# Edward-Sun/DIFUSCO

Hardware: AMD Instinct MI355X
Metric: denoising steps/sec (graphs x steps / s), TSP-1000 k-NN sparse categorical (higher is better)
Workload: dtype f32 (fp16x3 split MFMA, fp32 accumulate)

## Files before the change

difusco_amd/_lib.py:

```python
import ctypes
import os

from .build import LIB_PATH, PROF_LIB_PATH

FLAG_NO_L0_FOLD, FLAG_NO_TAIL_FOLD, FLAG_CHECK_FINITE = 1, 2, 4

ABI_VERSION = 13
TASK_TSP, TASK_MIS = 0, 1
CATEGORICAL, GAUSSIAN = 0, 1
RAND_NONE, RAND_INJECTED, RAND_PHILOX, RAND_PHILOX_INSTANCES = 0, 1, 2, 3
PREC_FP32, PREC_BF16X3, PREC_BF16X6, PREC_FP16X3, PREC_FP16X1 = 0, 1, 2, 3, 4
PRECISIONS = {"fp32": PREC_FP32, "bf16x3": PREC_BF16X3, "bf16x6": PREC_BF16X6, "fp16x3": PREC_FP16X3,
              "fp16x1": PREC_FP16X1}
FUSED_PRECISIONS = ("bf16x3", "fp16x3", "fp16x1")
GRAPH_PERM_IDENTITY, GRAPH_ORDER_IDENTITY, GRAPH_BAD_EDGE = 1, 2, 4
AGGREGATIONS = {"sum": 0, "mean": 1, "max": 2}

W_GLOBAL = ["node_embed.weight", "node_embed.bias", "edge_embed.weight", "edge_embed.bias",
            "time_embed.0.weight", "time_embed.0.bias", "time_embed.2.weight", "time_embed.2.bias",
            "out.0.weight", "out.0.bias", "out.2.weight", "out.2.bias",
            "@time_freqs", "@dimt_pos", "@dimt_scalar", "@planes:edge_embed.weight"]
W_LAYER = ["@node4.weight", "@node4.bias", "layers.{l}.C.weight", "layers.{l}.C.bias",
           "layers.{l}.norm_h.weight", "layers.{l}.norm_h.bias", "layers.{l}.norm_e.weight", "layers.{l}.norm_e.bias",
           "time_embed_layers.{l}.1.weight", "time_embed_layers.{l}.1.bias",
# ... 145 lines not shown
```

difusco_amd/csrc/api.hip:

```cpp
#include <hip/hip_runtime.h>

#include <cstdarg>
#include <cstdio>
#include <cstring>
#include <mutex>
#include <vector>

#include "../../include/difusco_hip.h"
#include "kernels.h"

namespace {

thread_local char g_err[512] = "";

int fail(int code, const char* fmt, ...) {
  va_list ap;
  va_start(ap, fmt);
  vsnprintf(g_err, sizeof(g_err), fmt, ap);
  va_end(ap);
  return code;
}

#define HIP_TRY(expr)                                                                         \
  do {                                                                                        \
// ... 195 lines not shown
  if (a->n_layers < 1) return fail(DIFUSCO_EINVAL, "n_layers must be >= 1");
  if (a->out_channels != 1 && a->out_channels != 2) return fail(DIFUSCO_EINVAL, "out_channels must be 1 or 2 (got %d)", a->out_channels);
  if (a->precision < DIFUSCO_PREC_FP32 || a->precision > DIFUSCO_PREC_FP16X1) return fail(DIFUSCO_EINVAL, "unknown precision %d", a->precision);
  return DIFUSCO_OK;
}

struct StepPlan {
  int H, L, C;
  int64_t N, E, out_rows, E_pad, n_tiles_pad;
  bool tsp, head_only;
  int nprec;
  bool f16;
  bool fused;
  int fused_variant;
  bool l0_fold, tail_fold, gn_fold, use_prep;
};

StepPlan make_plan(const difusco_step_args* a) {
  StepPlan p;
  p.H = a->hidden, p.L = a->n_layers, p.C = a->out_channels;
  p.N = a->n_nodes, p.E = a->n_edges;
  p.tsp = a->task == DIFUSCO_TASK_TSP;
  p.out_rows = p.tsp ? p.E : p.N;
  p.head_only = a->gn_phase == 2;
  p.nprec = a->precision == DIFUSCO_PREC_FP16X1 ? DIFUSCO_PREC_FP16X3 : a->precision;
  p.f16 = p.nprec == DIFUSCO_PREC_FP16X3;
  const int reg_gather = p.N >= (1 << 20) ? 1 : 0;
  const bool agg_max = a->aggregation == DIFUSCO_AGG_MAX;
  p.fused = p.H == 256 && !a->no_fusion && p.E > 0 && !(agg_max && reg_gather) &&
            (a->precision == DIFUSCO_PREC_BF16X3 || a->precision == DIFUSCO_PREC_FP16X3 ||
             a->precision == DIFUSCO_PREC_FP16X1);
  p.fused_variant = reg_gather | (agg_max ? 2 : 0);
  p.E_pad = (p.E + 255) / 256 * 256;
  p.n_tiles_pad = p.E_pad / 32;
#ifdef DIFUSCO_PROFILING
  const bool ablating = difusco::g_fused_ablate != 0;
#else
  const bool ablating = false;
#endif
  p.l0_fold = p.fused && (a->flags & DIFUSCO_FLAG_NO_L0_FOLD) == 0 && !ablating && (p.tsp ? a->xt_is_binary != 0 : true);
  p.tail_fold = p.fused && p.L >= 2 && (a->flags & DIFUSCO_FLAG_NO_TAIL_FOLD) == 0 && !ablating;
  p.gn_fold = p.tail_fold && p.tsp;
  p.use_prep = a->prepared != nullptr && p.fused && p.tsp && !ablating;
  return p;
}

hipError_t time_bias_rows(const Weights& w, int H, int L, const float* t_host, int n_t, float* out, hipStream_t st) {
  const int64_t* l0 = w.lo.off.data() + DIFUSCO_W_GLOBAL_COUNT;
  return difusco::launch_time_bias(t_host, n_t, H, L, w.g(DIFUSCO_W_TIME_FREQS), w.g(DIFUSCO_W_TIME0_W), w.g(DIFUSCO_W_TIME0_B),
                                   w.g(DIFUSCO_W_TIME2_W), w.g(DIFUSCO_W_TIME2_B), w.base + l0[0], w.lo.layer_stride,
                                   l0[DIFUSCO_WL_TIME_W] - l0[0], l0[DIFUSCO_WL_TIME_B] - l0[0], out, st);
}

int embed_tsp_nodes(const Weights& w, int H, int64_t N, const float* points, float* feat, float* h0, hipStream_t st, bool prof) {
  PROF_IF(prof, PROF_EMBED, launch_pos_embed(points, w.g(DIFUSCO_W_DIMT_POS), (int)N, H, feat, st))
  PROF_IF(prof, PROF_LINEAR_NODE, linear_rows(feat, w.g(DIFUSCO_W_NODE_EMBED_W), w.g(DIFUSCO_W_NODE_EMBED_B), nullptr, h0, N, H, H, H, st))
  return DIFUSCO_OK;
}

int node_rows(int precision, int H, int64_t N, const LayerW& lw, const float* h, float* hscale, bool scale_pass, bool fused_domain,
              float* dst, hipStream_t st, bool prof) {
  const int nprec = precision == DIFUSCO_PREC_FP16X1 ? DIFUSCO_PREC_FP16X3 : precision;
  const bool f16 = nprec == DIFUSCO_PREC_FP16X3;
  bool converted = false;
  if (precision != DIFUSCO_PREC_FP32 && H == 256) {
    const SplitPlanes np = split_planes(lw.node4_planes, 4 * H, H, f16);
    SplitScale sc;
    if (f16) {
      if (scale_pass) PROF_IF(prof, PROF_LINEAR_NODE, launch_row_pow2_scale(h, N, H, hscale, st))
      sc.row_scale = hscale;
      sc.w_inv = np.w_inv;
    }
    converted = fused_domain && (nprec == DIFUSCO_PREC_BF16X3 || nprec == DIFUSCO_PREC_FP16X3);
    if (converted) sc.w_inv = lw.node4_fused_s + (f16 ? 0 : 4 * H);
    PROF_IF(prof, PROF_LINEAR_NODE, linear_rows_split(h, np.planes, (long long)4 * H * H, nprec, converted ? lw.node4_fused_b : lw.node4_b,
                                                      nullptr, dst, N, H, 4 * H, 4 * H, st, 0, sc))
  } else {
    PROF_IF(prof, PROF_LINEAR_NODE, linear_rows(h, lw.node4_w, lw.node4_b, nullptr, dst, N, H, 4 * H, 4 * H, st))
  }
  if (fused_domain && !converted && H == 256) PROF_IF(prof, PROF_LINEAR_NODE, launch_fuse_node_tables(dst, lw.c_b, (int)N, dst, st))
  return DIFUSCO_OK;
}

hipError_t table_c_rows(int precision, int H, float* table, const LayerW& lw, float* scale2, hipStream_t st) {
  if (precision != DIFUSCO_PREC_FP16X1) return launch_two_rows_linear(H, table, lw.c_w, nullptr, table + 2 * H, st);
  hipError_t er = launch_row_pow2_scale(table, 2, H, scale2, st);
  if (er != hipSuccess) return er;
  const SplitPlanes cp = split_planes(lw.c_planes, H, H, true);
  SplitScale sc;
  sc.row_scale = scale2;
  sc.w_inv = cp.w_inv;
// ... 63 lines not shown
  }

  int embed_mis() const {
    PROF(PROF_EMBED, launch_scalar_embed(a->xt, nullptr, w.g(DIFUSCO_W_DIMT_SCALAR), p.N, H, ws.node4, st))
    PROF(PROF_LINEAR_NODE, linear_rows(ws.node4, w.g(DIFUSCO_W_NODE_EMBED_W), w.g(DIFUSCO_W_NODE_EMBED_B), nullptr, ws.h, p.N, H, H, H, st))
    if (p.l0_fold) {
      PROF(PROF_EMBED, zero_async(ws.table, sizeof(float) * 4 * H, st))
      PROF(PROF_EMBED, zero_pad_tail())
    } else if (p.E > 0) {
      PROF(PROF_EMBED, zero_async(ws.e, sizeof(float) * (p.fused ? p.E_pad : p.E) * H, st))
      if (p.fused && p.f16) PROF(PROF_EMBED, zero_async(ws.etmax, sizeof(float) * p.n_tiles_pad, st))
    }
    return DIFUSCO_OK;
  }

  int fused_layer(int l, const LayerW& lw, const float* node4, const float* h_in) const {
    const float* tb = tbias + (size_t)l * H;
    FusedLayerArgs fa;
    fa.e = ws.e, fa.node4 = node4, fa.row = a->row, fa.col = a->col, fa.n_edges = (int)p.E;
    fa.c_planes = split_planes(lw.c_planes, H, H, p.f16).planes;
    fa.o_planes = split_planes(lw.out_planes, H, H, p.f16).planes;
    fa.plane_stride = (long long)H * H;
    fa.b_c = lw.c_b, fa.g_e = lw.norm_e_w, fa.b_e = lw.norm_e_b, fa.tbias = tb;
    fa.g_o = lw.out_ln_w, fa.b_o = lw.out_ln_b, fa.b_out = lw.out_b;
    fa.time_on_edge = p.tsp ? 1 : 0;
    fa.part = ws.part, fa.direct = ws.direct, fa.scales = lw.fused_scales, fa.stream = st;
    FusedKind kind = FusedKind::Middle;
    if (l == 0 && p.l0_fold) {
      kind = FusedKind::FirstFromTable;
      fa.l0_table = table, fa.l0_x = p.tsp ? a->xt : nullptr, fa.l0_perm = p.tsp ? a->perm : nullptr;
      fa.etmax_out = ws.etmax;
    } else if (p.tail_fold && l == p.L - 1) {
      kind = p.tsp ? FusedKind::TailTsp : FusedKind::TailMis;
      fa.gn_tile = ws.gn_tile, fa.etmax_in = ws.etmax;
    } else {
      fa.etmax_in = fa.etmax_out = ws.etmax;
    }
    PROF(PROF_LINEAR_EDGE, launch_edge_layer_fused(a->precision, kind, p.fused_variant, fa))
    if (p.gn_fold && l == p.L - 1) return DIFUSCO_OK;
#ifdef DIFUSCO_PROFILING
    if (g_step_skip & 1) return DIFUSCO_OK;
#endif
    PROF(PROF_GATE, launch_node_finalize((int)p.N, (int)p.E, a->rowptr, node4, ws.part, ws.direct, ws.h, lw.norm_h_w, lw.norm_h_b, tb,
                                         p.tsp ? 1 : 0, p.f16 ? ws.hscale : nullptr, st, h_in, a->aggregation))
    return DIFUSCO_OK;
  }

  int unfused_layer(int l, const LayerW& lw) const {
    PROF(PROF_LINEAR_EDGE, edge_linear(a->precision, ws.e, lw.c_w, lw.c_planes, lw.c_b, nullptr, ws.tmp))
    PROF(PROF_GATE, launch_edge_gate_aggregate(H, (int)p.N, a->rowptr, a->col, ws.node4, ws.tmp, ws.h, lw.norm_h_w, lw.norm_h_b,
                                               lw.norm_e_w, lw.norm_e_b, lw.out_ln_w, lw.out_ln_b, tbias + (size_t)l * H,
                                               p.tsp ? 1 : 0, st, a->aggregation))
    PROF(PROF_LINEAR_EDGE, edge_linear(a->precision, ws.tmp, lw.out_w, lw.out_planes, lw.out_b, ws.e, ws.e))
    return DIFUSCO_OK;
  }

  int run_layers() const {
    for (int l = 0; l < p.L; ++l) {
      const LayerW lw = w.layer(l);
      const bool prep_l = p.use_prep && l == 0;
      bool node_linear = !prep_l;
#ifdef DIFUSCO_PROFILING
      if ((g_step_skip & 2) && l >= 2) node_linear = false;
#endif
      if (node_linear)
        STAGE(node_rows(a->precision, H, p.N, lw, ws.h, ws.hscale, !p.fused || l == 0, p.fused, ws.node4, st, true));
      STAGE(p.fused ? fused_layer(l, lw, prep_l ? prep.node4_0 : ws.node4, prep_l ? prep.h0 : nullptr) : unfused_layer(l, lw));
    }
    return DIFUSCO_OK;
  }

  int run_head(const uint64_t* offset_shift) const {
    RandInstances ri;
    if (a->rand_mode == DIFUSCO_RAND_PHILOX_INSTANCES) ri = RandInstances{a->n_instances, a->instance_rows, a->instance_seeds};
    const int* seg_ptr = a->n_segments > 1 ? a->seg_ptr : nullptr;
    const int nblk = gn_blocks_for(p.out_rows);
    if (p.fused && p.tsp) {
      PROF(PROF_HEAD, launch_head_tiled(p.C, ws.e, p.E, nblk < 8 ? 8 : nblk / 8 * 8, ws.partial, ws.stats, w.g(DIFUSCO_W_OUT_GN_W),
                                        w.g(DIFUSCO_W_OUT_GN_B), w.g(DIFUSCO_W_OUT_CONV_W), w.g(DIFUSCO_W_OUT_CONV_B), a->perm, a->xt,
                                        a->post, a->rand_mode, a->rand, a->seed, a->offset, a->xt_out, a->pred_out, a->prob_out, st,
                                        p.gn_fold ? ws.gn_tile : nullptr, a->gn_phase, a->gn_sums, seg_ptr, a->n_segments, ri,
                                        offset_shift))
      return DIFUSCO_OK;
    }
    PROF(PROF_HEAD, launch_head(H, p.C, p.tsp ? ws.e : ws.h, seg_ptr, a->n_segments, p.out_rows, nblk, ws.partial, ws.stats,
                                w.g(DIFUSCO_W_OUT_GN_W), w.g(DIFUSCO_W_OUT_GN_B), w.g(DIFUSCO_W_OUT_CONV_W), w.g(DIFUSCO_W_OUT_CONV_B),
                                p.tsp ? a->perm : nullptr, a->xt, a->post, a->rand_mode, a->rand, a->seed, a->offset, a->xt_out,
                                a->pred_out, a->prob_out, st, a->gn_phase, a->gn_sums, ri, offset_shift))
    return DIFUSCO_OK;
  }

  int check_finite() const {
    if ((a->flags & DIFUSCO_FLAG_CHECK_FINITE) == 0 || a->gn_phase == 1) return DIFUSCO_OK;
    unsigned* cnt = reinterpret_cast<unsigned*>(ws.partial);
    HIP_TRY(hipMemsetAsync(cnt, 0, sizeof(unsigned), st));
    HIP_TRY(launch_count_nonfinite(a->xt_out, p.out_rows, cnt, st));
    HIP_TRY(launch_count_nonfinite(ws.stats, (long long)a->n_segments * 64, cnt, st));
// ... 382 lines not shown
```

difusco_amd/csrc/graph_kernels.hip:

```cpp
#include "common.h"
#include "kernels.h"

namespace difusco {

template <int VEC>
struct Vec {
  float v[VEC];
};

template <int VEC>
__device__ __forceinline__ Vec<VEC> ldv(const float* p) {
  Vec<VEC> r;
  if constexpr (VEC == 4) {
    const v4f t = *reinterpret_cast<const v4f*>(p);
    r.v[0] = t[0]; r.v[1] = t[1]; r.v[2] = t[2]; r.v[3] = t[3];
  } else if constexpr (VEC == 2) {
    typedef float v2f __attribute__((ext_vector_type(2)));
    const v2f t = *reinterpret_cast<const v2f*>(p);
    r.v[0] = t[0]; r.v[1] = t[1];
  } else {
    r.v[0] = *p;
  }
  return r;
}
// ... 212 lines not shown
  }
  s += __shfl_xor(s, 1, 64);
  q += __shfl_xor(q, 1, 64);
  if ((lane & 1) == 0) {
    red[wave][lane >> 1][0] = s;
    red[wave][lane >> 1][1] = q;
  }
  __syncthreads();
  if (threadIdx.x < 64) {
    const int g = threadIdx.x >> 1, w = threadIdx.x & 1;
    const double t = red[0][g][w] + red[1][g][w] + red[2][g][w] + red[3][g][w];
    partial[((long long)seg * gridDim.x + blockIdx.x) * 64 + g * 2 + w] = t;
  }
}

__global__ __launch_bounds__(1024) void gn_finalize_kernel(const double* __restrict__ partial, const int* __restrict__ seg_ptr,
                                                          long long total_rows, int nblk, int ch_per_group,
                                                          int group_stride_blocks, float* __restrict__ stats,
                                                          double* __restrict__ sums_out) {
  __shared__ double red[16][64];
  const int seg = blockIdx.x;
  const int c = threadIdx.x >> 6, gw = threadIdx.x & 63, g = gw >> 1, nch = blockDim.x >> 6;
  double acc = 0.0;
  if (group_stride_blocks == 1) {
    for (int b = c; b < nblk; b += nch) acc += partial[((long long)seg * nblk + b) * 64 + gw];
  } else {
    for (int b = (g >> 2) + 8 * c; b < nblk; b += 8 * nch) acc += partial[((long long)seg * nblk + b) * 64 + gw];
  }
  red[c][gw] = acc;
  __syncthreads();
  if (threadIdx.x < 32) {
    const int gg = threadIdx.x;
    double s = 0.0, q = 0.0;
    for (int k = 0; k < nch; ++k) {
      s += red[k][2 * gg];
      q += red[k][2 * gg + 1];
    }
    const long long rows = seg_ptr ? (long long)(seg_ptr[seg + 1] - seg_ptr[seg]) : total_rows;
    if (sums_out) {
      sums_out[2 * gg] = s;
      sums_out[2 * gg + 1] = q;
      if (gg == 0) sums_out[64] = (double)rows;
      return;
    }
    const double cnt = (double)rows * ch_per_group;
    const double mean = s / cnt;
    double var = q / cnt - mean * mean;
    var = var > 0.0 ? var : 0.0;
    stats[(seg * 32 + gg) * 2 + 0] = (float)mean;
    stats[(seg * 32 + gg) * 2 + 1] = (float)(1.0 / sqrt(var + 1e-5));
  }
}

__global__ void gn_stats_from_sums_kernel(const double* __restrict__ sums, int ch_per_group, float* __restrict__ stats) {
  const int gg = threadIdx.x;
  if (gg >= 32) return;
  const double cnt = sums[64] * ch_per_group;
  const double mean = sums[2 * gg] / cnt;
  double var = sums[2 * gg + 1] / cnt - mean * mean;
  var = var > 0.0 ? var : 0.0;
  stats[gg * 2 + 0] = (float)mean;
  stats[gg * 2 + 1] = (float)(1.0 / sqrt(var + 1e-5));
}

struct PostParams {
// ... 227 lines not shown
      s[k] += __shfl_xor(s[k], off, 64);
      q[k] += __shfl_xor(q[k], off, 64);
    }
  }
  if (lane == 0) {
    double* dst = partial + ((long long)seg * gridDim.x + blockIdx.x) * 64 + 16 * wave;
#pragma unroll
    for (int k = 0; k < 8; ++k) {
      dst[2 * k] = s[k];
      dst[2 * k + 1] = q[k];
    }
  }
}

__global__ __launch_bounds__(256) void gn_tiles_reduce_kernel(const float* __restrict__ gn_tile, long long n_tiles, long long rows,
                                                              double* __restrict__ partial) {
  __shared__ double red[4][64];
  const int c = threadIdx.x & 63, r = threadIdx.x >> 6;
  double acc = 0.0;
  for (long long t = (long long)blockIdx.x * 4 + r; t < n_tiles; t += (long long)gridDim.x * 4) {
    const float* src = gn_tile + t * 96;
    const long long left = rows - t * 32;
    const double n = 8.0 * (double)(left < 32 ? left : 32);
    const double p = (double)src[64 + (c >> 1)], sd = (double)src[c & ~1];
    acc += (c & 1) ? (double)src[c] + 2.0 * p * sd + n * p * p : sd + n * p;
  }
  red[r][c] = acc;
  __syncthreads();
  if (r == 0) partial[(long long)blockIdx.x * 64 + c] = ((red[0][c] + red[1][c]) + red[2][c]) + red[3][c];
}

template <int C, bool SEG>
__global__ __launch_bounds__(256) void head_apply_tiled_kernel(const float* __restrict__ feat, long long rows,
                                                               long long n_tiles, const float* __restrict__ stats,
                                                               const float* __restrict__ gn_w, const float* __restrict__ gn_b,
                                                               const float* __restrict__ conv_w, const float* __restrict__ conv_b,
                                                               const int* __restrict__ perm, const float* __restrict__ xt,
                                                               PostParams pp, float* __restrict__ xt_out,
                                                               float* __restrict__ pred_out, float* __restrict__ prob_out,
                                                               const int* __restrict__ seg_ptr, int n_segments) {
  __shared__ float st[64];
  __shared__ __attribute__((aligned(16))) float s_gw[256], s_gb[256], s_cw[C][256];
  if (threadIdx.x < 64) st[threadIdx.x] = stats[threadIdx.x];
  s_gw[threadIdx.x] = gn_w[threadIdx.x];
// ... 258 lines not shown
    y[H + f] = a1 + b;
  }
}

hipError_t launch_two_rows_linear(int H, const float* x, const float* w, const float* bias, float* y, hipStream_t stream) {
  dim3 grid((unsigned)(H / 4));
  DIFUSCO_VEC_DISPATCH(H, hipLaunchKernelGGL((two_rows_linear_kernel<VEC>), grid, dim3(256), 0, stream, x, w, bias, y))
  return hipGetLastError();
}

hipError_t launch_head_tiled(int C, const float* feat, long long rows, int nblk, double* partial, float* stats,
                             const float* gn_w, const float* gn_b, const float* conv_w, const float* conv_b,
                             const int* perm, const float* xt, const float* post, int rand_mode, const float* rand,
                             unsigned long long seed, unsigned long long offset, float* xt_out, float* pred_out,
                             float* prob_out, hipStream_t stream, const float* gn_tile, int gn_phase, double* gn_sums,
                             const int* seg_ptr, int n_segments, RandInstances ri, const uint64_t* offset_shift) {
  if (rows == 0) return hipSuccess;
  if (gn_phase != 0 && !gn_sums) return hipErrorInvalidValue;
  if (n_segments > 1) {
    if (!seg_ptr || gn_phase != 0) return hipErrorInvalidValue;
    const PostParams pq = make_post(post, rand_mode, rand, seed, offset, ri, offset_shift);
    const long long n_tiles_s = (rows + 31) / 32;
    int bps = (int)((n_tiles_s / n_segments + 3) / 4);
    bps = bps < 1 ? 1 : (bps > 256 ? 256 : bps);
    hipLaunchKernelGGL(gn_partial_tiled_seg_kernel, dim3(bps, n_segments), dim3(256), 0, stream, feat, seg_ptr, partial);
    hipLaunchKernelGGL(gn_finalize_kernel, dim3(n_segments), dim3(1024), 0, stream, partial, seg_ptr, rows, bps, 8, 1, stats,
                       (double*)nullptr);
    long long blocks_s = (n_tiles_s + 3) / 4;
    if (blocks_s > 4096) blocks_s = 4096;
    if (C == 2) {
      hipLaunchKernelGGL((head_apply_tiled_kernel<2, true>), dim3((unsigned)blocks_s), dim3(256), 0, stream, feat, rows, n_tiles_s,
// ... 1 lines not shown
    } else if (C == 1) {
      hipLaunchKernelGGL((head_apply_tiled_kernel<1, true>), dim3((unsigned)blocks_s), dim3(256), 0, stream, feat, rows, n_tiles_s,
                         stats, gn_w, gn_b, conv_w, conv_b, perm, xt, pq, xt_out, pred_out, prob_out, seg_ptr, n_segments);
    } else {
      return hipErrorInvalidValue;
    }
    return hipGetLastError();
  }
  if (nblk < 8 || nblk % 8 != 0) return hipErrorInvalidValue;
  const PostParams pp = make_post(post, rand_mode, rand, seed, offset, ri, offset_shift);
  const long long n_tiles = (rows + 31) / 32;
  double* sums_out = gn_phase == 1 ? gn_sums : (double*)nullptr;
  if (gn_phase == 2) {
    hipLaunchKernelGGL(gn_stats_from_sums_kernel, dim3(1), dim3(64), 0, stream, gn_sums, 8, stats);
  } else if (gn_tile) {
    hipLaunchKernelGGL(gn_tiles_reduce_kernel, dim3(256), dim3(256), 0, stream, gn_tile, n_tiles, rows, partial);
    hipLaunchKernelGGL(gn_finalize_kernel, dim3(1), dim3(1024), 0, stream, partial, (const int*)nullptr, rows, 256, 8, 1, stats,
                       sums_out);
  } else {
    hipLaunchKernelGGL(gn_partial_tiled_kernel, dim3(nblk), dim3(256), 0, stream, feat, n_tiles, partial);
    hipLaunchKernelGGL(gn_finalize_kernel, dim3(1), dim3(1024), 0, stream, partial, (const int*)nullptr, rows, nblk, 8, 8, stats,
                       sums_out);
  }
  if (gn_phase == 1) return hipGetLastError();
  long long blocks = (n_tiles + 3) / 4;
  if (blocks > 4096) blocks = 4096;
  if (C == 2) {
    hipLaunchKernelGGL((head_apply_tiled_kernel<2, false>), dim3((unsigned)blocks), dim3(256), 0, stream, feat, rows, n_tiles, stats,
                       gn_w, gn_b, conv_w, conv_b, perm, xt, pp, xt_out, pred_out, prob_out, (const int*)nullptr, 1);
  } else if (C == 1) {
    hipLaunchKernelGGL((head_apply_tiled_kernel<1, false>), dim3((unsigned)blocks), dim3(256), 0, stream, feat, rows, n_tiles, stats,
                       gn_w, gn_b, conv_w, conv_b, perm, xt, pp, xt_out, pred_out, prob_out, (const int*)nullptr, 1);
  } else {
// ... 7 lines not shown
```

difusco_amd/csrc/kernels.h:

```cpp
#pragma once
#include <hip/hip_runtime.h>

#include <atomic>

namespace difusco {

inline hipError_t ensure_max_dynamic_lds(std::atomic<unsigned long long>& devices, const void* fn, int bytes) {
  int dev = 0;
  hipError_t er = hipGetDevice(&dev);
  if (er != hipSuccess) return er;
  const unsigned long long bit = 1ull << (dev & 63);
  if (devices.load(std::memory_order_acquire) & bit) return hipSuccess;
  er = hipFuncSetAttribute(fn, hipFuncAttributeMaxDynamicSharedMemorySize, bytes);
  if (er != hipSuccess) return er;
  devices.fetch_or(bit, std::memory_order_release);
  return hipSuccess;
}

int set_error(int code, const char* fmt, ...);

__host__ __device__ inline long long edge_tiled_offset(long long s, int f) {
  return (s >> 5) * 8192 + (long long)(f >> 4) * 512 + ((f >> 3) & 1) * 256 + ((((f >> 2) & 1) * 32) + (s & 31)) * 4 + (f & 3);
}

hipError_t linear_rows(const float* x, const float* w, const float* bias, const float* residual, float* y,
                       long long m, int k, int n_out, long long ldy, hipStream_t stream);

struct SplitScale {
  const float* row_scale = nullptr;
  float x_scale = 1.0f;
  const float* w_inv = nullptr;
  float* tile_max = nullptr;
};

hipError_t linear_rows_split(const float* x, const unsigned short* wp, long long plane_stride, int mode,
                             const float* bias, const float* residual, float* y, long long m, int k, int n_out,
                             long long ldy, hipStream_t stream, int tiled_out = 0, SplitScale sc = SplitScale());

hipError_t node_linear(const float* x, const float* row_scale, long long m, const unsigned short* planes, long long plane_stride,
                       int mode, int n_out, const float* w_inv, const float* bias, float* y, hipStream_t stream);

hipError_t linear_scalar_embed_split(const float* x, const int* perm, const float* dimt, const unsigned short* wp,
                                     long long plane_stride, int mode, const float* bias, float* y, long long m,
                                     hipStream_t stream, int tiled_out, const float* w_inv, float* tile_max);

hipError_t launch_edge_embed_tiled(const float* x, const int* perm, const float* dimt, const unsigned short* planes, long long plane_stride,
                                   int mode, const float* w_inv, const float* bias, float* e, long long n_edges, float* tile_max,
                                   hipStream_t stream, const float* gen_table = nullptr, int* tile_flag = nullptr);
constexpr float kGenXMin = -8.0f, kGenH = 0.25f, kGenInvH = 4.0f;
constexpr int kGenIntervals = 64, kGenRows = kGenIntervals + 7;
hipError_t launch_gen_table_grid(float* x, hipStream_t stream);

hipError_t launch_row_pow2_scale(const float* x, long long m, int k, float* scale, hipStream_t stream);
hipError_t launch_count_nonfinite(const float* x, long long n, unsigned* count, hipStream_t stream);
hipError_t launch_zero_words(void* p, size_t bytes, hipStream_t stream);
// ... 49 lines not shown
hipError_t launch_table_rows(const float* x, const int* perm, const float* table, long long rows, int H, float* out,
                             hipStream_t stream);
hipError_t launch_table_rows_tiled(const float* x, const int* perm, const float* table, long long rows, float* out,
                                   hipStream_t stream);
struct RandInstances {
  int n = 0;
  const int64_t* rows = nullptr;
  const uint64_t* seeds = nullptr;
};
hipError_t launch_head_tiled(int C, const float* feat, long long rows, int nblk, double* partial, float* stats,
                             const float* gn_w, const float* gn_b, const float* conv_w, const float* conv_b,
                             const int* perm, const float* xt, const float* post, int rand_mode, const float* rand,
                             unsigned long long seed, unsigned long long offset, float* xt_out, float* pred_out,
                             float* prob_out, hipStream_t stream, const float* gn_tile = nullptr, int gn_phase = 0,
                             double* gn_sums = nullptr, const int* seg_ptr = nullptr, int n_segments = 1,
                             RandInstances ri = RandInstances{}, const uint64_t* offset_shift = nullptr);
hipError_t launch_edge_gate_aggregate(int H, int n_nodes, const int* rowptr, const int* col, const float* node4,
                                      float* ce_act, float* h, const float* nh_w, const float* nh_b, const float* ne_w,
                                      const float* ne_b, const float* ol_w, const float* ol_b, const float* tbias,
                                      int time_on_edge, hipStream_t stream, int agg_mode = 0);
int gn_blocks_for(long long rows);
hipError_t launch_head(int H, int C, const float* feat, const int* seg_ptr, int n_segments, long long total_rows,
                       int nblk, double* partial, float* stats, const float* gn_w, const float* gn_b,
                       const float* conv_w, const float* conv_b, const int* perm, const float* xt, const float* post,
                       int rand_mode, const float* rand, unsigned long long seed, unsigned long long offset,
                       float* xt_out, float* pred_out, float* prob_out, hipStream_t stream, int gn_phase = 0,
                       double* gn_sums = nullptr, RandInstances ri = RandInstances{},
                       const uint64_t* offset_shift = nullptr);
hipError_t launch_categorical_posterior(const float* logits, const float* xt, const float* post, int rand_mode,
                                        const float* rand, unsigned long long seed, unsigned long long offset,
                                        float* xt_out, float* prob_out, long long n, hipStream_t stream);
// ... 6 lines not shown
```

difusco_amd/csrc/linear_split.hip:

```cpp
#include <type_traits>

#include "common.h"
#include "kernels.h"

namespace difusco {

typedef __bf16 v8bf __attribute__((ext_vector_type(8)));
typedef __bf16 v2bf __attribute__((ext_vector_type(2)));
typedef float v2f __attribute__((ext_vector_type(2)));
typedef unsigned int v2u __attribute__((ext_vector_type(2)));
typedef unsigned int v4u __attribute__((ext_vector_type(4)));

typedef _Float16 v8h __attribute__((ext_vector_type(8)));
typedef _Float16 v2h __attribute__((ext_vector_type(2)));

struct Bf16 {
  typedef v8bf frag;
  __device__ static __forceinline__ unsigned split_pair(float& a, float& b) {
    v2f f = {a, b};
    v2bf h = __builtin_convertvector(f, v2bf);
    a -= (float)h[0];
    b -= (float)h[1];
    return __builtin_bit_cast(unsigned, h);
  }
// ... 210 lines not shown
  if (D > 1) grid = dim3((unsigned)(8 * (((m + 127) / 128 + 7) / 8) * (n_out / FB)), 1);
  hipLaunchKernelGGL((linear_rows_split_kernel<K, FB, NS, T, GEN, D>), grid, dim3(256), lds, stream, x, wp, plane_stride, n_out,
                     bias, residual, y, m, ldy, tiled_out, gen_perm, gen_dimt, row_scale, x_scale, w_inv, tile_max);
  return hipGetLastError();
}

#ifdef DIFUSCO_PROFILING
int g_node_linear_depth = 0;
#define NODE_LINEAR_DEPTH g_node_linear_depth
#else
#define NODE_LINEAR_DEPTH 0
#endif

hipError_t linear_rows_split(const float* x, const unsigned short* wp, long long plane_stride, int mode,
                             const float* bias, const float* residual, float* y, long long m, int k, int n_out,
                             long long ldy, hipStream_t stream, int tiled_out, SplitScale sc) {
  if (m <= 0) return hipSuccess;
  if (mode < 1 || mode > 4) return hipErrorInvalidValue;
  if (tiled_out && (k != 256 || n_out != 256 || residual != nullptr)) return hipErrorInvalidValue;
  if (sc.tile_max != nullptr && !tiled_out) return hipErrorInvalidValue;
#define DIFUSCO_SPLIT_ARGS x, wp, plane_stride, bias, residual, y, m, n_out, ldy, stream, tiled_out, nullptr, nullptr, sc.row_scale, sc.x_scale, sc.w_inv, sc.tile_max
#define DIFUSCO_SPLIT_CASE(KK, FBB)                                                   \
  if (k == KK && n_out % FBB == 0) {                                                  \
    if (mode == 1) return launch_split<KK, FBB, 2, Bf16>(DIFUSCO_SPLIT_ARGS);         \
    if (mode == 2) return launch_split<KK, FBB, 3, Bf16>(DIFUSCO_SPLIT_ARGS);         \
    if (mode == 4) return launch_split<KK, FBB, 1, Fp16>(DIFUSCO_SPLIT_ARGS);         \
    return launch_split<KK, FBB, 2, Fp16>(DIFUSCO_SPLIT_ARGS);                        \
  }
  if (k == 256 && !tiled_out && n_out % 128 == 0 && ((m + 127) / 128) * (n_out / 256) < 512) {
    if (NODE_LINEAR_DEPTH == 0 && (mode == 1 || mode == 3) && residual == nullptr && ldy == n_out && sc.x_scale == 1.0f &&
        (mode == 1 || (sc.row_scale != nullptr && sc.w_inv != nullptr)))
      return node_linear(x, sc.row_scale, m, wp, plane_stride, mode, n_out, sc.w_inv, bias, y, stream);
    if (NODE_LINEAR_DEPTH != 1) {
      if (mode == 1) return launch_split<256, 128, 2, Bf16, false, 4>(DIFUSCO_SPLIT_ARGS);
      if (mode == 3) return launch_split<256, 128, 2, Fp16, false, 4>(DIFUSCO_SPLIT_ARGS);
    }
    DIFUSCO_SPLIT_CASE(256, 128)
  }
  DIFUSCO_SPLIT_CASE(256, 256)
  DIFUSCO_SPLIT_CASE(128, 128)
  DIFUSCO_SPLIT_CASE(64, 64)
#undef DIFUSCO_SPLIT_CASE
#undef DIFUSCO_SPLIT_ARGS
  return hipErrorInvalidValue;
}

hipError_t linear_scalar_embed_split(const float* x, const int* perm, const float* dimt, const unsigned short* wp,
// ... 35 lines not shown
```

difusco_amd/csrc/node_linear.hip:

```cpp
#include "edge_layer_common.h"

namespace difusco {

namespace nodelin {
constexpr int K = 256, RB = 128, CB = 128, NSLAB = K / 16;
constexpr int SPS = 2;
constexpr int NSTAGE = NSLAB / SPS;
constexpr int NBUF = 3;
constexpr int PLANE = CB * 16;
constexpr int BUF = SPS * 2 * PLANE;
}

template <typename T, int ABL = 0>
__global__ __launch_bounds__(256, 2) void node_linear_kernel(const float* __restrict__ X, long long M,
                                                             const float* __restrict__ row_scale,
                                                             const unsigned short* __restrict__ planes, long long plane_stride,
                                                             int n_out, const float* __restrict__ w_inv,
                                                             const float* __restrict__ bias, float* __restrict__ Y) {
  using namespace nodelin;
  typedef typename T::frag frag;
  __shared__ __attribute__((aligned(16))) unsigned short wbuf[NBUF * BUF];
  const int tid = threadIdx.x, lane = tid & 63, l31 = lane & 31, hh = lane >> 5;
  const int wave = __builtin_amdgcn_readfirstlane(tid >> 6);
  const int ncb = n_out / CB, slot = (int)blockIdx.x >> 3;
  const int rb_i = (slot / ncb) * 8 + ((int)blockIdx.x & 7), cb_i = slot % ncb;
  if ((long long)rb_i * RB >= M) return;
  const long long row_raw = (long long)rb_i * RB + wave * 32 + l31;
  const long long row = row_raw < M ? row_raw : M - 1;
  const int f0 = cb_i * CB;

  const __amdgpu_buffer_rsrc_t rs_w = __builtin_amdgcn_make_buffer_rsrc(const_cast<unsigned short*>(planes), 0, 0x7fffffff, 0x00020000);
  const int plane_bytes = (int)plane_stride * 2;
  unsigned dvoff;
  {
    const int entry = wave * 32 + (lane >> 1), half = (lane & 1) ^ ((lane >> 4) & 1);
    dvoff = (unsigned)((f0 + entry) * 32 + half * 16);
  }
#define NODELIN_DMA_STAGE(t)                                                                                            \
  {                                                                                                                     \
    _Pragma("unroll") for (int sl = 0; sl < SPS; ++sl)                                                                  \
    _Pragma("unroll") for (int pl = 0; pl < 2; ++pl)                                                                    \
      __builtin_amdgcn_raw_ptr_buffer_load_lds(rs_w,                                                                    \
          (__attribute__((address_space(3))) void*)(wbuf + ((t) % NBUF) * BUF + (sl * 2 + pl) * PLANE + wave * 512), 16, \
          dvoff, (SPS * (t) + sl) * n_out * 32 + pl * plane_bytes, 0, 0);                                               \
// ... 127 lines not shown
    for (int r = 0; r < 16; ++r) {
      const int m = 8 * (r >> 2) + (r & 3);
      if (full || rbase + 4 * hh + m < M) {
#pragma unroll
        for (int nb = 0; nb < 4; ++nb) yb[(long long)m * n_out + nb * 32] = acc[nb][r] * (wv[nb] * rs[r]) + bv[nb];
      }
    }
  }
}

#ifdef DIFUSCO_PROFILING
int g_node_linear_ablate = 0;
#endif

hipError_t node_linear(const float* x, const float* row_scale, long long m, const unsigned short* planes, long long plane_stride,
                       int mode, int n_out, const float* w_inv, const float* bias, float* y, hipStream_t stream) {
  using namespace nodelin;
  if (m <= 0) return hipSuccess;
  if (n_out % CB != 0 || (mode != 1 && mode != 3) || (mode == 3 && (row_scale == nullptr || w_inv == nullptr))) return hipErrorInvalidValue;
  const unsigned grid = (unsigned)(8 * (((m + RB - 1) / RB + 7) / 8) * (n_out / CB));
#ifdef DIFUSCO_PROFILING
#define NODELIN_ABL_CASE(A)                                                                                                        \
  if (g_node_linear_ablate == A) {                                                                                                 \
    hipLaunchKernelGGL((node_linear_kernel<FFp16, A>), dim3(grid), dim3(256), 0, stream, x, m, row_scale, planes, plane_stride,    \
                       n_out, w_inv, bias, y);                                                                                     \
    return hipGetLastError();                                                                                                      \
  }
  if (mode == 3) {
    NODELIN_ABL_CASE(1) NODELIN_ABL_CASE(2) NODELIN_ABL_CASE(3) NODELIN_ABL_CASE(4) NODELIN_ABL_CASE(5) NODELIN_ABL_CASE(7) NODELIN_ABL_CASE(16)
  }
#undef NODELIN_ABL_CASE
#endif
  if (mode == 3)
    hipLaunchKernelGGL((node_linear_kernel<FFp16>), dim3(grid), dim3(256), 0, stream, x, m, row_scale, planes, plane_stride, n_out, w_inv,
                       bias, y);
  else
    hipLaunchKernelGGL((node_linear_kernel<FBf16>), dim3(grid), dim3(256), 0, stream, x, m, row_scale, planes, plane_stride, n_out, w_inv,
                       bias, y);
  return hipGetLastError();
}

}
```

include/difusco_hip.h:

```cpp
#ifndef DIFUSCO_HIP_H
#define DIFUSCO_HIP_H

#include <stddef.h>
#include <stdint.h>

#ifdef __cplusplus
extern "C" {
#endif

#define DIFUSCO_ABI_VERSION 13

enum {
  DIFUSCO_OK = 0,
  DIFUSCO_EINVAL = -1,
  DIFUSCO_EWORKSPACE = -2,
  DIFUSCO_EHIP = -3,
  DIFUSCO_EUNSUPPORTED = -4,
  DIFUSCO_ENONFINITE = -5
};

enum { DIFUSCO_TASK_TSP = 0, DIFUSCO_TASK_MIS = 1 };
enum { DIFUSCO_CATEGORICAL = 0, DIFUSCO_GAUSSIAN = 1 };
enum { DIFUSCO_AGG_SUM = 0, DIFUSCO_AGG_MEAN = 1, DIFUSCO_AGG_MAX = 2 };
enum {
// ... 96 lines not shown
  int32_t flags;
  double* gn_sums;
  const void* prepared;
  const float* tbias;
  int32_t aggregation;
  int32_t reserved0;
  const float* gen_table;
  int32_t n_instances;
  const int64_t* instance_rows;
  const uint64_t* instance_seeds;
} difusco_step_args;

enum {
  DIFUSCO_FLAG_NO_L0_FOLD = 1,
  DIFUSCO_FLAG_NO_TAIL_FOLD = 2,
  DIFUSCO_FLAG_CHECK_FINITE = 4
};

size_t difusco_workspace_bytes(int hidden, int n_layers, int n_nodes, int n_edges, int n_segments);

size_t difusco_prepared_bytes(int hidden, int n_nodes);
int difusco_prepare(const difusco_step_args* args, void* prepared, size_t prepared_bytes);
int difusco_time_bias_rows(int hidden, int n_layers, int out_channels, const float* weights, const float* t_host, int n_t,
                           float* out, void* stream);

int difusco_edge_embed(int hidden, int n_layers, int out_channels, const float* weights, int precision, const float* xt,
                       const int32_t* perm, int64_t n_edges, float* e_tiled, float* tile_max, const float* gen_table, void* stream);

size_t difusco_gen_table_bytes(int hidden);
int difusco_gen_table_build(int hidden, int n_layers, int out_channels, const float* weights, float* table, size_t table_bytes,
// ... 127 lines not shown
```

Baseline: 891.1.

## Compute only A|B node columns in last layer and fold GN finalize into reduce

In the last fused TSP layer only the edge update runs, so the node linear now computes just the A and B column blocks (half of the 4H outputs) instead of all four. Separately, the group-norm tile reduction gains a last-block-arrives pattern with a global atomic counter, so the final block computes the stats and the separate single-block finalize kernel launch is skipped. This removes a chunk of GEMM work and one kernel launch per step. In exchange it adds a device-global arrival counter keyed by buffer address, which falls back when the stream is capturing or no slot is available, and relies on careful memory ordering.

```diff
diff --git a/difusco_amd/_lib.py b/difusco_amd/_lib.py
--- a/difusco_amd/_lib.py
+++ b/difusco_amd/_lib.py
@@ -3,7 +3,7 @@
 
 from .build import LIB_PATH, PROF_LIB_PATH
 
-FLAG_NO_L0_FOLD, FLAG_NO_TAIL_FOLD, FLAG_CHECK_FINITE = 1, 2, 4
+FLAG_NO_L0_FOLD, FLAG_NO_TAIL_FOLD, FLAG_CHECK_FINITE, FLAG_NO_NODE_FOLD = 1, 2, 4, 8
 
 ABI_VERSION = 13
 TASK_TSP, TASK_MIS = 0, 1
diff --git a/difusco_amd/csrc/api.hip b/difusco_amd/csrc/api.hip
--- a/difusco_amd/csrc/api.hip
+++ b/difusco_amd/csrc/api.hip
@@ -233,6 +233,7 @@
   bool fused;
   int fused_variant;
   bool l0_fold, tail_fold, gn_fold, use_prep;
+  bool node_fold;
 };
 
 StepPlan make_plan(const difusco_step_args* a) {
@@ -260,6 +261,7 @@
   p.l0_fold = p.fused && (a->flags & DIFUSCO_FLAG_NO_L0_FOLD) == 0 && !ablating && (p.tsp ? a->xt_is_binary != 0 : true);
   p.tail_fold = p.fused && p.L >= 2 && (a->flags & DIFUSCO_FLAG_NO_TAIL_FOLD) == 0 && !ablating;
   p.gn_fold = p.tail_fold && p.tsp;
+  p.node_fold = p.gn_fold && (a->flags & DIFUSCO_FLAG_NO_NODE_FOLD) == 0;
   p.use_prep = a->prepared != nullptr && p.fused && p.tsp && !ablating;
   return p;
 }
@@ -278,7 +280,7 @@
 }
 
 int node_rows(int precision, int H, int64_t N, const LayerW& lw, const float* h, float* hscale, bool scale_pass, bool fused_domain,
-              float* dst, hipStream_t st, bool prof) {
+              float* dst, hipStream_t st, bool prof, bool ab_only = false) {
   const int nprec = precision == DIFUSCO_PREC_FP16X1 ? DIFUSCO_PREC_FP16X3 : precision;
   const bool f16 = nprec == DIFUSCO_PREC_FP16X3;
   bool converted = false;
@@ -292,8 +294,9 @@
     }
     converted = fused_domain && (nprec == DIFUSCO_PREC_BF16X3 || nprec == DIFUSCO_PREC_FP16X3);
     if (converted) sc.w_inv = lw.node4_fused_s + (f16 ? 0 : 4 * H);
+    const int col0 = ab_only && converted ? 2 * H : 0;
     PROF_IF(prof, PROF_LINEAR_NODE, linear_rows_split(h, np.planes, (long long)4 * H * H, nprec, converted ? lw.node4_fused_b : lw.node4_b,
-                                                      nullptr, dst, N, H, 4 * H, 4 * H, st, 0, sc))
+                                                      nullptr, dst, N, H, 4 * H, 4 * H, st, 0, sc, col0, col0 ? 2 * H : 0))
   } else {
     PROF_IF(prof, PROF_LINEAR_NODE, linear_rows(h, lw.node4_w, lw.node4_b, nullptr, dst, N, H, 4 * H, 4 * H, st))
   }
@@ -387,7 +390,7 @@
     return DIFUSCO_OK;
   }
 
-  int fused_layer(int l, const LayerW& lw, const float* node4, const float* h_in) const {
+  int fused_layer(int l, const LayerW& lw, const float* node4, const float* h_in, bool node4_ab_only) const {
     const float* tb = tbias + (size_t)l * H;
     FusedLayerArgs fa;
     fa.e = ws.e, fa.node4 = node4, fa.row = a->row, fa.col = a->col, fa.n_edges = (int)p.E;
@@ -409,8 +412,10 @@
     } else {
       fa.etmax_in = fa.etmax_out = ws.etmax;
     }
+    if (node4_ab_only && kind != FusedKind::TailTsp) return fail(DIFUSCO_EINVAL, "internal: V gathers from an A | B-only node4");
     PROF(PROF_LINEAR_EDGE, launch_edge_layer_fused(a->precision, kind, p.fused_variant, fa))
     if (p.gn_fold && l == p.L - 1) return DIFUSCO_OK;
+    if (node4_ab_only) return fail(DIFUSCO_EINVAL, "internal: node update from an A | B-only node4");
 #ifdef DIFUSCO_PROFILING
     if (g_step_skip & 1) return DIFUSCO_OK;
 #endif
@@ -436,9 +441,10 @@
 #ifdef DIFUSCO_PROFILING
       if ((g_step_skip & 2) && l >= 2) node_linear = false;
 #endif
+      const bool ab_only = node_linear && p.node_fold && l == p.L - 1;
       if (node_linear)
-        STAGE(node_rows(a->precision, H, p.N, lw, ws.h, ws.hscale, !p.fused || l == 0, p.fused, ws.node4, st, true));
-      STAGE(p.fused ? fused_layer(l, lw, prep_l ? prep.node4_0 : ws.node4, prep_l ? prep.h0 : nullptr) : unfused_layer(l, lw));
+        STAGE(node_rows(a->precision, H, p.N, lw, ws.h, ws.hscale, !p.fused || l == 0, p.fused, ws.node4, st, true, ab_only));
+      STAGE(p.fused ? fused_layer(l, lw, prep_l ? prep.node4_0 : ws.node4, prep_l ? prep.h0 : nullptr, ab_only) : unfused_layer(l, lw));
     }
     return DIFUSCO_OK;
   }
@@ -453,7 +459,7 @@
                                         w.g(DIFUSCO_W_OUT_GN_B), w.g(DIFUSCO_W_OUT_CONV_W), w.g(DIFUSCO_W_OUT_CONV_B), a->perm, a->xt,
                                         a->post, a->rand_mode, a->rand, a->seed, a->offset, a->xt_out, a->pred_out, a->prob_out, st,
                                         p.gn_fold ? ws.gn_tile : nullptr, a->gn_phase, a->gn_sums, seg_ptr, a->n_segments, ri,
-                                        offset_shift))
+                                        offset_shift, p.node_fold))
       return DIFUSCO_OK;
     }
     PROF(PROF_HEAD, launch_head(H, p.C, p.tsp ? ws.e : ws.h, seg_ptr, a->n_segments, p.out_rows, nblk, ws.partial, ws.stats,
diff --git a/difusco_amd/csrc/graph_kernels.hip b/difusco_amd/csrc/graph_kernels.hip
--- a/difusco_amd/csrc/graph_kernels.hip
+++ b/difusco_amd/csrc/graph_kernels.hip
@@ -1,3 +1,6 @@
+#include <mutex>
+#include <unordered_map>
+
 #include "common.h"
 #include "kernels.h"
 
@@ -250,6 +253,27 @@
   }
 }
 
+__device__ __forceinline__ void gn_stats_of_group(double (*red)[64], int nch, int gg, long long rows, int ch_per_group,
+                                                  float* __restrict__ stats, double* __restrict__ sums_out) {
+  double s = 0.0, q = 0.0;
+  for (int k = 0; k < nch; ++k) {
+    s += red[k][2 * gg];
+    q += red[k][2 * gg + 1];
+  }
+  if (sums_out) {
+    sums_out[2 * gg] = s;
+    sums_out[2 * gg + 1] = q;
+    if (gg == 0) sums_out[64] = (double)rows;
+    return;
+  }
+  const double cnt = (double)rows * ch_per_group;
+  const double mean = s / cnt;
+  double var = q / cnt - mean * mean;
+  var = var > 0.0 ? var : 0.0;
+  stats[gg * 2 + 0] = (float)mean;
+  stats[gg * 2 + 1] = (float)(1.0 / sqrt(var + 1e-5));
+}
+
 __global__ __launch_bounds__(1024) void gn_finalize_kernel(const double* __restrict__ partial, const int* __restrict__ seg_ptr,
                                                           long long total_rows, int nblk, int ch_per_group,
                                                           int group_stride_blocks, float* __restrict__ stats,
@@ -266,25 +290,8 @@
   red[c][gw] = acc;
   __syncthreads();
   if (threadIdx.x < 32) {
-    const int gg = threadIdx.x;
-    double s = 0.0, q = 0.0;
-    for (int k = 0; k < nch; ++k) {
-      s += red[k][2 * gg];
-      q += red[k][2 * gg + 1];
-    }
     const long long rows = seg_ptr ? (long long)(seg_ptr[seg + 1] - seg_ptr[seg]) : total_rows;
-    if (sums_out) {
-      sums_out[2 * gg] = s;
-      sums_out[2 * gg + 1] = q;
-      if (gg == 0) sums_out[64] = (double)rows;
-      return;
-    }
-    const double cnt = (double)rows * ch_per_group;
-    const double mean = s / cnt;
-    double var = q / cnt - mean * mean;
-    var = var > 0.0 ? var : 0.0;
-    stats[(seg * 32 + gg) * 2 + 0] = (float)mean;
-    stats[(seg * 32 + gg) * 2 + 1] = (float)(1.0 / sqrt(var + 1e-5));
+    gn_stats_of_group(red, nch, threadIdx.x, rows, ch_per_group, stats + seg * 64, sums_out);
   }
 }
 
@@ -542,8 +549,10 @@
 }
 
 __global__ __launch_bounds__(256) void gn_tiles_reduce_kernel(const float* __restrict__ gn_tile, long long n_tiles, long long rows,
-                                                              double* __restrict__ partial) {
-  __shared__ double red[4][64];
+                                                              double* partial, unsigned* arrivals, float* __restrict__ stats,
+                                                              double* __restrict__ sums_out) {
+  __shared__ double red[16][64];
+  __shared__ int is_last;
   const int c = threadIdx.x & 63, r = threadIdx.x >> 6;
   double acc = 0.0;
   for (long long t = (long long)blockIdx.x * 4 + r; t < n_tiles; t += (long long)gridDim.x * 4) {
@@ -555,7 +564,64 @@
   }
   red[r][c] = acc;
   __syncthreads();
-  if (r == 0) partial[(long long)blockIdx.x * 64 + c] = ((red[0][c] + red[1][c]) + red[2][c]) + red[3][c];
+  const double row_sum = ((red[0][c] + red[1][c]) + red[2][c]) + red[3][c];
+  if (arrivals == nullptr) {
+    if (r == 0) partial[(long long)blockIdx.x * 64 + c] = row_sum;
+    return;
+  }
+  if (r == 0) {
+    __hip_atomic_store(partial + (long long)blockIdx.x * 64 + c, row_sum, __ATOMIC_RELAXED, __HIP_MEMORY_SCOPE_AGENT);
+    asm volatile("s_waitcnt vmcnt(0)" ::: "memory");
+    if (threadIdx.x == 0) {
+      const unsigned ticket = __hip_atomic_fetch_add(arrivals, 1u, __ATOMIC_RELAXED, __HIP_MEMORY_SCOPE_AGENT);
+      const int last = ticket == gridDim.x - 1;
+      if (last) {
+        __hip_atomic_store(arrivals, 0u, __ATOMIC_RELAXED, __HIP_MEMORY_SCOPE_AGENT);
+        __builtin_amdgcn_fence(__ATOMIC_ACQUIRE, "agent");
+        asm volatile("s_waitcnt vmcnt(0)" ::: "memory");
+      }
+      is_last = last;
+    }
+  }
+  __syncthreads();
+  if (!is_last) return;
+  const int nblk = (int)gridDim.x;
+#pragma unroll
+  for (int k = 0; k < 4; ++k) {
+    const int ch = r + 4 * k;
+    double a = 0.0;
+#pragma unroll 8
+    for (int b = ch; b < nblk; b += 16) a += partial[(long long)b * 64 + c];
+    red[ch][c] = a;
+  }
+  __syncthreads();
+  if (threadIdx.x < 32) gn_stats_of_group(red, 16, threadIdx.x, rows, 8, stats, sums_out);
+}
+
+constexpr int GN_ARRIVAL_SLOTS = 4096;
+__device__ unsigned g_gn_arrivals[GN_ARRIVAL_SLOTS];
+
+static unsigned* gn_arrival_counter(const void* partial, hipStream_t stream) {
+  static std::mutex mu;
+  static std::unordered_map<const void*, int> slot_of;
+  static std::unordered_map<int, unsigned*> base_of_device;
+  std::lock_guard<std::mutex> lk(mu);
+  int dev = 0;
+  if (hipGetDevice(&dev) != hipSuccess) return nullptr;
+  auto bd = base_of_device.find(dev);
+  if (bd == base_of_device.end()) {
+    hipStreamCaptureStatus cap = hipStreamCaptureStatusNone;
+    if (hipStreamIsCapturing(stream, &cap) != hipSuccess || cap != hipStreamCaptureStatusNone) return nullptr;
+    void* p = nullptr;
+    if (hipGetSymbolAddress(&p, HIP_SYMBOL(g_gn_arrivals)) != hipSuccess) return nullptr;
+    bd = base_of_device.emplace(dev, static_cast<unsigned*>(p)).first;
+  }
+  auto it = slot_of.find(partial);
+  if (it == slot_of.end()) {
+    if ((int)slot_of.size() >= GN_ARRIVAL_SLOTS) return nullptr;
+    it = slot_of.emplace(partial, (int)slot_of.size()).first;
+  }
+  return bd->second + it->second;
 }
 
 template <int C, bool SEG>
@@ -844,7 +910,8 @@
                              const int* perm, const float* xt, const float* post, int rand_mode, const float* rand,
                              unsigned long long seed, unsigned long long offset, float* xt_out, float* pred_out,
                              float* prob_out, hipStream_t stream, const float* gn_tile, int gn_phase, double* gn_sums,
-                             const int* seg_ptr, int n_segments, RandInstances ri, const uint64_t* offset_shift) {
+                             const int* seg_ptr, int n_segments, RandInstances ri, const uint64_t* offset_shift,
+                             bool fold_stats) {
   if (rows == 0) return hipSuccess;
   if (gn_phase != 0 && !gn_sums) return hipErrorInvalidValue;
   if (n_segments > 1) {
@@ -876,9 +943,12 @@
   if (gn_phase == 2) {
     hipLaunchKernelGGL(gn_stats_from_sums_kernel, dim3(1), dim3(64), 0, stream, gn_sums, 8, stats);
   } else if (gn_tile) {
-    hipLaunchKernelGGL(gn_tiles_reduce_kernel, dim3(256), dim3(256), 0, stream, gn_tile, n_tiles, rows, partial);
-    hipLaunchKernelGGL(gn_finalize_kernel, dim3(1), dim3(1024), 0, stream, partial, (const int*)nullptr, rows, 256, 8, 1, stats,
+    unsigned* arrivals = fold_stats ? gn_arrival_counter(partial, stream) : nullptr;
+    hipLaunchKernelGGL(gn_tiles_reduce_kernel, dim3(256), dim3(256), 0, stream, gn_tile, n_tiles, rows, partial, arrivals, stats,
                        sums_out);
+    if (arrivals == nullptr)
+      hipLaunchKernelGGL(gn_finalize_kernel, dim3(1), dim3(1024), 0, stream, partial, (const int*)nullptr, rows, 256, 8, 1, stats,
+                         sums_out);
   } else {
     hipLaunchKernelGGL(gn_partial_tiled_kernel, dim3(nblk), dim3(256), 0, stream, feat, n_tiles, partial);
     hipLaunchKernelGGL(gn_finalize_kernel, dim3(1), dim3(1024), 0, stream, partial, (const int*)nullptr, rows, nblk, 8, 8, stats,
diff --git a/difusco_amd/csrc/kernels.h b/difusco_amd/csrc/kernels.h
--- a/difusco_amd/csrc/kernels.h
+++ b/difusco_amd/csrc/kernels.h
@@ -35,10 +35,12 @@
 
 hipError_t linear_rows_split(const float* x, const unsigned short* wp, long long plane_stride, int mode,
                              const float* bias, const float* residual, float* y, long long m, int k, int n_out,
-                             long long ldy, hipStream_t stream, int tiled_out = 0, SplitScale sc = SplitScale());
+                             long long ldy, hipStream_t stream, int tiled_out = 0, SplitScale sc = SplitScale(), int col0 = 0,
+                             int n_cols = 0);
 
 hipError_t node_linear(const float* x, const float* row_scale, long long m, const unsigned short* planes, long long plane_stride,
-                       int mode, int n_out, const float* w_inv, const float* bias, float* y, hipStream_t stream);
+                       int mode, int n_out, const float* w_inv, const float* bias, float* y, hipStream_t stream, int col0 = 0,
+                       int n_cols = 0);
 
 hipError_t linear_scalar_embed_split(const float* x, const int* perm, const float* dimt, const unsigned short* wp,
                                      long long plane_stride, int mode, const float* bias, float* y, long long m,
@@ -118,7 +120,8 @@
                              unsigned long long seed, unsigned long long offset, float* xt_out, float* pred_out,
                              float* prob_out, hipStream_t stream, const float* gn_tile = nullptr, int gn_phase = 0,
                              double* gn_sums = nullptr, const int* seg_ptr = nullptr, int n_segments = 1,
-                             RandInstances ri = RandInstances{}, const uint64_t* offset_shift = nullptr);
+                             RandInstances ri = RandInstances{}, const uint64_t* offset_shift = nullptr,
+                             bool fold_stats = false);
 hipError_t launch_edge_gate_aggregate(int H, int n_nodes, const int* rowptr, const int* col, const float* node4,
                                       float* ce_act, float* h, const float* nh_w, const float* nh_b, const float* ne_w,
                                       const float* ne_b, const float* ol_w, const float* ol_b, const float* tbias,
diff --git a/difusco_amd/csrc/linear_split.hip b/difusco_amd/csrc/linear_split.hip
--- a/difusco_amd/csrc/linear_split.hip
+++ b/difusco_amd/csrc/linear_split.hip
@@ -248,9 +248,10 @@
 
 hipError_t linear_rows_split(const float* x, const unsigned short* wp, long long plane_stride, int mode,
                              const float* bias, const float* residual, float* y, long long m, int k, int n_out,
-                             long long ldy, hipStream_t stream, int tiled_out, SplitScale sc) {
+                             long long ldy, hipStream_t stream, int tiled_out, SplitScale sc, int col0, int n_cols) {
   if (m <= 0) return hipSuccess;
   if (mode < 1 || mode > 4) return hipErrorInvalidValue;
+  if (col0 < 0 || n_cols < 0 || col0 % 128 != 0 || n_cols % 128 != 0 || col0 + n_cols > n_out) return hipErrorInvalidValue;
   if (tiled_out && (k != 256 || n_out != 256 || residual != nullptr)) return hipErrorInvalidValue;
   if (sc.tile_max != nullptr && !tiled_out) return hipErrorInvalidValue;
 #define DIFUSCO_SPLIT_ARGS x, wp, plane_stride, bias, residual, y, m, n_out, ldy, stream, tiled_out, nullptr, nullptr, sc.row_scale, sc.x_scale, sc.w_inv, sc.tile_max
@@ -264,7 +265,7 @@
   if (k == 256 && !tiled_out && n_out % 128 == 0 && ((m + 127) / 128) * (n_out / 256) < 512) {
     if (NODE_LINEAR_DEPTH == 0 && (mode == 1 || mode == 3) && residual == nullptr && ldy == n_out && sc.x_scale == 1.0f &&
         (mode == 1 || (sc.row_scale != nullptr && sc.w_inv != nullptr)))
-      return node_linear(x, sc.row_scale, m, wp, plane_stride, mode, n_out, sc.w_inv, bias, y, stream);
+      return node_linear(x, sc.row_scale, m, wp, plane_stride, mode, n_out, sc.w_inv, bias, y, stream, col0, n_cols);
     if (NODE_LINEAR_DEPTH != 1) {
       if (mode == 1) return launch_split<256, 128, 2, Bf16, false, 4>(DIFUSCO_SPLIT_ARGS);
       if (mode == 3) return launch_split<256, 128, 2, Fp16, false, 4>(DIFUSCO_SPLIT_ARGS);
diff --git a/difusco_amd/csrc/node_linear.hip b/difusco_amd/csrc/node_linear.hip
--- a/difusco_amd/csrc/node_linear.hip
+++ b/difusco_amd/csrc/node_linear.hip
@@ -15,19 +15,20 @@
 __global__ __launch_bounds__(256, 2) void node_linear_kernel(const float* __restrict__ X, long long M,
                                                              const float* __restrict__ row_scale,
                                                              const unsigned short* __restrict__ planes, long long plane_stride,
-                                                             int n_out, const float* __restrict__ w_inv,
+                                                             int n_out, int col0, int n_cols,
+                                                             const float* __restrict__ w_inv,
                                                              const float* __restrict__ bias, float* __restrict__ Y) {
   using namespace nodelin;
   typedef typename T::frag frag;
   __shared__ __attribute__((aligned(16))) unsigned short wbuf[NBUF * BUF];
   const int tid = threadIdx.x, lane = tid & 63, l31 = lane & 31, hh = lane >> 5;
   const int wave = __builtin_amdgcn_readfirstlane(tid >> 6);
-  const int ncb = n_out / CB, slot = (int)blockIdx.x >> 3;
+  const int ncb = n_cols / CB, slot = (int)blockIdx.x >> 3;
   const int rb_i = (slot / ncb) * 8 + ((int)blockIdx.x & 7), cb_i = slot % ncb;
   if ((long long)rb_i * RB >= M) return;
   const long long row_raw = (long long)rb_i * RB + wave * 32 + l31;
   const long long row = row_raw < M ? row_raw : M - 1;
-  const int f0 = cb_i * CB;
+  const int f0 = col0 + cb_i * CB;
 
   const __amdgpu_buffer_rsrc_t rs_w = __builtin_amdgcn_make_buffer_rsrc(const_cast<unsigned short*>(planes), 0, 0x7fffffff, 0x00020000);
   const int plane_bytes = (int)plane_stride * 2;
@@ -185,16 +186,19 @@
 #endif
 
 hipError_t node_linear(const float* x, const float* row_scale, long long m, const unsigned short* planes, long long plane_stride,
-                       int mode, int n_out, const float* w_inv, const float* bias, float* y, hipStream_t stream) {
+                       int mode, int n_out, const float* w_inv, const float* bias, float* y, hipStream_t stream, int col0,
+                       int n_cols) {
   using namespace nodelin;
   if (m <= 0) return hipSuccess;
+  if (n_cols == 0) n_cols = n_out - col0;
+  if (col0 < 0 || n_cols <= 0 || col0 % CB != 0 || n_cols % CB != 0 || col0 + n_cols > n_out) return hipErrorInvalidValue;
   if (n_out % CB != 0 || (mode != 1 && mode != 3) || (mode == 3 && (row_scale == nullptr || w_inv == nullptr))) return hipErrorInvalidValue;
-  const unsigned grid = (unsigned)(8 * (((m + RB - 1) / RB + 7) / 8) * (n_out / CB));
+  const unsigned grid = (unsigned)(8 * (((m + RB - 1) / RB + 7) / 8) * (n_cols / CB));
 #ifdef DIFUSCO_PROFILING
 #define NODELIN_ABL_CASE(A)                                                                                                        \
   if (g_node_linear_ablate == A) {                                                                                                 \
     hipLaunchKernelGGL((node_linear_kernel<FFp16, A>), dim3(grid), dim3(256), 0, stream, x, m, row_scale, planes, plane_stride,    \
-                       n_out, w_inv, bias, y);                                                                                     \
+                       n_out, col0, n_cols, w_inv, bias, y);                                                                       \
     return hipGetLastError();                                                                                                      \
   }
   if (mode == 3) {
@@ -203,11 +207,11 @@
 #undef NODELIN_ABL_CASE
 #endif
   if (mode == 3)
-    hipLaunchKernelGGL((node_linear_kernel<FFp16>), dim3(grid), dim3(256), 0, stream, x, m, row_scale, planes, plane_stride, n_out, w_inv,
-                       bias, y);
+    hipLaunchKernelGGL((node_linear_kernel<FFp16>), dim3(grid), dim3(256), 0, stream, x, m, row_scale, planes, plane_stride, n_out, col0,
+                       n_cols, w_inv, bias, y);
   else
-    hipLaunchKernelGGL((node_linear_kernel<FBf16>), dim3(grid), dim3(256), 0, stream, x, m, row_scale, planes, plane_stride, n_out, w_inv,
-                       bias, y);
+    hipLaunchKernelGGL((node_linear_kernel<FBf16>), dim3(grid), dim3(256), 0, stream, x, m, row_scale, planes, plane_stride, n_out, col0,
+                       n_cols, w_inv, bias, y);
   return hipGetLastError();
 }
 
diff --git a/include/difusco_hip.h b/include/difusco_hip.h
--- a/include/difusco_hip.h
+++ b/include/difusco_hip.h
@@ -134,6 +134,7 @@
 enum {
   DIFUSCO_FLAG_NO_L0_FOLD = 1,
   DIFUSCO_FLAG_NO_TAIL_FOLD = 2,
+  DIFUSCO_FLAG_NO_NODE_FOLD = 8,
   DIFUSCO_FLAG_CHECK_FINITE = 4
 };
 
```

Result: no change. 892.0 (median of 2 runs) (+0.1%).
